# pySTEPS/pysteps

Hardware: AMD Instinct MI355X
Metric: Mpixels*leadsteps/s (LK+semilag) at 4096x4096 fp32 (higher is better)
Workload: dtype f32

## Files before the change

pysteps_amd/csrc/semilag.hip:

```cpp
#include <algorithm>
#include <cstdio>
#include <cstdlib>
#include <cstring>
#include <vector>

#include "common.h"

#pragma clang fp contract(off)

#include "semilag_device.h"

namespace psh {
namespace {

using namespace sl;

constexpr int kTileX = 64;
enum : int { kModeDirect = 0, kModePacked = 3, kModePacked2 = 4 };
constexpr int kDirectWaves = 8;
struct Fields {
  const float *u0, *v0, *p0;
  __amdgpu_buffer_rsrc_t ru, rv, rp;
  __amdgpu_buffer_rsrc_t ruv;
  __amdgpu_buffer_rsrc_t rpp;
// ... 353 lines not shown
        for (int j = 0; j < NPX; ++j) {
          mx[j] = px[j];
          my[j] = py[j];
          gx[j] = fx[j];
          gy[j] = fy[j];
          retreat(mx[j], gx[j], vix[j]);
          retreat(my[j], gy[j], viy[j]);
        }
        sample_at<NPX, ORDER, kVel, MODE, GEN>(F, mx, my, gx, gy, m, n, outval, su, sv, sp);
#pragma unroll
        for (int j = 0; j < NPX; ++j) {
          retreat(px[j], fx[j], su[j] * s);
          retreat(py[j], fy[j], sv[j] * s);
        }
        if (HAS_PRECIP && k == n_iter - 1) {
          sample_at<NPX, ORDER, kVel | kPrecip, MODE, GEN>(F, px, py, fx, fy, m, n, outval, su, sv, sp);
        } else {
          sample_at<NPX, ORDER, kVel, MODE, GEN>(F, px, py, fx, fy, m, n, outval, su, sv, sp);
        }
#pragma unroll
        for (int j = 0; j < NPX; ++j) {
          vix[j] = su[j] * half_s;
          viy[j] = sv[j] * half_s;
        }
      }
    } else {
      if (t > 0 || resume == 1) {
        sample_at<NPX, ORDER, kVel, MODE, GEN>(F, px, py, fx, fy, m, n, outval, su, sv, sp);
#pragma unroll
        for (int j = 0; j < NPX; ++j) {
          vix[j] = su[j] * s;
          viy[j] = sv[j] * s;
        }
      }
#pragma unroll
      for (int j = 0; j < NPX; ++j) {
        retreat(px[j], fx[j], vix[j]);
        retreat(py[j], fy[j], viy[j]);
      }
      if (HAS_PRECIP) {
        bool inside = true;
#pragma unroll
        for (int j = 0; j < NPX; ++j) inside = inside && wave_all_interior(px[j], py[j], m, n);
        if (ORDER == 1 && inside) {
          float v[NPX][4];
#pragma unroll
          for (int j = 0; j < NPX; ++j) {
            const unsigned off = static_cast<unsigned>(__mul24(py[j], n) + px[j]) << 2;
            v[j][0] = ld(F.p0, off);
            v[j][1] = ld(F.p0, off, 1);
            v[j][2] = ld(F.p0, off + static_cast<unsigned>(F.row_bytes));
            v[j][3] = ld(F.p0, off + static_cast<unsigned>(F.row_bytes), 1);
          }
#pragma unroll
          for (int j = 0; j < NPX; ++j)
            sp[j] = blend(make_weights(fx[j], fy[j]), v[j][0], v[j][1], v[j][2], v[j][3]);
          asm volatile("" ::: "memory");
        } else {
#pragma unroll
          for (int j = 0; j < NPX; ++j)
            sp[j] = ORDER == 3
                        ? sample_cubic<GEN>(F, px[j], py[j], fx[j], fy[j], m, n, outval)
                        : sample_precip_off_fast<(ORDER == 3 ? 1 : ORDER), GEN>(F.p0, px[j], py[j], fx[j], fy[j], m,
                                                                       n, outval, F.bmode);
        }
      }
    }
    if (HAS_PRECIP) {
#pragma unroll
      for (int j = 0; j < NPX; ++j) {
        sp[j] = lost(fx[j], fy[j]) ? lostval : sp[j];
        if (live[j]) {
          __builtin_nontemporal_store(sp[j], reinterpret_cast<float *>(reinterpret_cast<char *>(out) + opix[j]));
        }
      }
      out += static_cast<size_t>(rows) * n;
    }
  }

  if (disp != nullptr) {
#pragma unroll
    for (int j = 0; j < NPX; ++j) {
      if (!live[j]) continue;
      disp[static_cast<size_t>(y[j]) * n + x] =
          static_cast<double>(px[j]) - static_cast<double>(x) + static_cast<double>(fx[j]);
      disp[plane + static_cast<size_t>(y[j]) * n + x] =
          static_cast<double>(py[j]) - static_cast<double>(y[j]) + static_cast<double>(fy[j]);
    }
  }
}


typedef __attribute__((address_space(3))) void lds_void;
typedef __attribute__((address_space(3))) float lds_f32;
typedef __attribute__((address_space(3))) u32x4 lds_u32x4;
typedef __attribute__((address_space(3))) int lds_int;

__device__ __forceinline__ void win_barrier() { asm volatile("s_waitcnt lgkmcnt(0)\n\ts_barrier" ::: "memory"); }

__device__ __forceinline__ int rfl(int v) { return __builtin_amdgcn_readfirstlane(v); }

__device__ __forceinline__ int smin(int a, int b) {
  int r;
  asm("s_min_i32 %0, %1, %2" : "=s"(r) : "s"(a), "s"(b) : "scc");
  return r;
}
__device__ __forceinline__ int smax(int a, int b) {
  int r;
  asm("s_max_i32 %0, %1, %2" : "=s"(r) : "s"(a), "s"(b) : "scc");
  return r;
}

static unsigned long long *g_win_stats = nullptr;

template <int WAVES, int WW, int WH, int ROWS = 4, int OCC = 4>
struct WinCfg {
  static constexpr int kWaves = WAVES, kW = WW, kH = WH;
  static constexpr int kRows = ROWS;
  static constexpr int kOcc = OCC;
  static constexpr int kTileY = ROWS * WAVES;
  static constexpr unsigned kPitch4 = WW * 4u;
  static constexpr unsigned kPlaneBytes = WW * WH * 4u;
  static constexpr int kItems = WH * (WW / 4);
  static constexpr int kThreads = kTileX * WAVES;
  static constexpr unsigned kCtlVel = 16u * WAVES, kCtlFlag = kCtlVel + 8u;
  static constexpr unsigned kCtlTile = kCtlFlag + 12u;
  static constexpr int kCtlWords = 4 * WAVES + 2 + 3 + 3;
};
using Win8 = WinCfg<8, 96, 64>;

struct Window {
  unsigned uv, p;
  unsigned ctl;
  int ox, oy;
  int lo_x, hi_x, lo_y, hi_y;
  int edge;
  int fill16;
  unsigned long long *stats;
};

__device__ __forceinline__ void win_count(const Window &W, int which) {
  if (W.stats != nullptr && (threadIdx.x & 63) == 0) atomicAdd(W.stats + which, 1ull);
}

struct WinBox {
  int lox, hix, loy, hiy;
};
template <int kWinRows>
__device__ __forceinline__ WinBox win_corners(const int (&dxw)[kWinRows], const int (&dy)[kWinRows]) {
  const int xa = __builtin_amdgcn_readlane(dxw[0], 0), xb = __builtin_amdgcn_readlane(dxw[0], 63);
  const int xc = __builtin_amdgcn_readlane(dxw[kWinRows - 1], 0), xd = __builtin_amdgcn_readlane(dxw[kWinRows - 1], 63);
  const int ya = __builtin_amdgcn_readlane(dy[0], 0), yb = __builtin_amdgcn_readlane(dy[0], 63);
  const int yc = __builtin_amdgcn_readlane(dy[kWinRows - 1], 0), yd = __builtin_amdgcn_readlane(dy[kWinRows - 1], 63);
  return {smin(smin(xa, xb), smin(xc, xd)), smax(smax(xa, xb), smax(xc, xd)), smin(smin(ya, yb), smin(yc, yd)),
          smax(smax(ya, yb), smax(yc, yd))};
}

template <class C>
__device__ __forceinline__ void win_publish(const Window &W, int wave, const WinBox &bx, float vx_lane, float vy_lane) {
  typedef int i32x4 __attribute__((ext_vector_type(4)));
  typedef __attribute__((address_space(3))) i32x4 lds_i32x4;
  lds_int *ctl = (lds_int *)(size_t)W.ctl;
  *(lds_i32x4 *)(size_t)(W.ctl + 16u * wave) = i32x4{bx.lox, bx.hix, bx.loy, bx.hiy};
  if (wave == 0) {
    ctl[C::kCtlVel / 4 + 0] = __float_as_int(vx_lane);
    ctl[C::kCtlVel / 4 + 1] = __float_as_int(vy_lane);
  }
}

template <class C, bool GEN>
__device__ __forceinline__ void win_place_and_fill(const Fields &F, Window &W, bool force, int (&dxw)[C::kRows],
                                                    int (&dy)[C::kRows], float move_scale, int m, int n) {
  constexpr int kWinRows = C::kRows;
  lds_int *ctl = (lds_int *)(size_t)W.ctl;
  int ulox = 0x7fffffff, uhix = -0x7fffffff, uloy = 0x7fffffff, uhiy = -0x7fffffff;
#pragma unroll
  for (int w = 0; w < C::kWaves; ++w) {
    ulox = min(ulox, ctl[w * 4 + 0]);
    uhix = max(uhix, ctl[w * 4 + 1]);
    uloy = min(uloy, ctl[w * 4 + 2]);
    uhiy = max(uhiy, ctl[w * 4 + 3]);
  }
  const float wvx = __int_as_float(ctl[C::kCtlVel / 4 + 0]), wvy = __int_as_float(ctl[C::kCtlVel / 4 + 1]);
  const int bx0 = ulox, bx1 = uhix + 1, by0 = uloy, by1 = uhiy + 1;
  const int slack_x = max(C::kW - (bx1 - bx0 + 1), 0), slack_y = max(C::kH - (by1 - by0 + 1), 0);
  const int keep_x = wvx > 0.125f ? max(slack_x - 2, 0) : (wvx < -0.125f ? min(slack_x, 2) : slack_x / 2);
  const int keep_y = wvy > 0.125f ? max(slack_y - 2, 0) : (wvy < -0.125f ? min(slack_y, 2) : slack_y / 2);
  constexpr int kFar = 1 << 27;
  const int want_x = min(max(sat_add(W.ox, sat_sub(bx0, keep_x)), -kFar), kFar) & ~3;
  const int want_y = min(max(sat_add(W.oy, sat_sub(by0, keep_y)), -kFar), kFar);
  const int nox = rfl(GEN ? min(max(want_x, 0), n - C::kW) : want_x);
  const int noy = rfl(GEN ? min(max(want_y, 0), m - C::kH) : want_y);
  const bool edge = !GEN && (nox < 0 || nox + C::kW > n || noy < 0 || noy + C::kH > m);
  PSH_DASSERT((W.fill16 == 0 || (nox & 3) == 0) && (edge || (nox >= 0 && nox + C::kW <= n && noy >= 0 && noy + C::kH <= m)));
  const float mvx = fabsf(wvx) < 64.f ? fabsf(wvx) * move_scale + 2.f : 2.f, mvy = fabsf(wvy) < 64.f ? fabsf(wvy) * move_scale + 2.f : 2.f;
  const int gx = rfl(static_cast<int>(mvx)), gy = rfl(static_cast<int>(mvy));
  W.lo_x = wvx > 0.f ? gx : 1;
  W.hi_x = C::kW - 2 - (wvx > 0.f ? 1 : gx);
  W.lo_y = wvy > 0.f ? gy : 1;
  W.hi_y = C::kH - 2 - (wvy > 0.f ? 1 : gy);
  if (!force && nox == W.ox && noy == W.oy) return;
  win_count(W, 2);
  const int ddx = nox - W.ox, ddy = noy - W.oy;
#pragma unroll
  for (int j = 0; j < kWinRows; ++j) {
    dxw[j] = sat_sub(dxw[j], ddx);
    dy[j] = sat_sub(dy[j], ddy);
  }
  W.ox = nox;
  W.oy = noy;
  W.edge = edge ? 1 : 0;
  int tid = threadIdx.x;
  asm volatile("" : "+v"(tid));
  constexpr int kRounds = (C::kItems + C::kThreads - 1) / C::kThreads;
  u32x4 bu[kRounds], bv[kRounds], bp[kRounds];
  if (!edge) {
    const unsigned org = static_cast<unsigned>(noy) * static_cast<unsigned>(n) + static_cast<unsigned>(nox);
#pragma unroll
    for (int k = 0; k < kRounds; ++k) {
      const int item = min(tid + C::kThreads * k, C::kItems - 1);
      const int row = item / (C::kW / 4), c = item - row * (C::kW / 4);
      const int off = static_cast<int>((org + row * n + 4 * c) << 2);
      bu[k] = __builtin_amdgcn_raw_buffer_load_b128(F.ru, off, 0, 0);
      bv[k] = __builtin_amdgcn_raw_buffer_load_b128(F.rv, off, 0, 0);
      bp[k] = __builtin_amdgcn_raw_buffer_load_b128(F.rp, off, 0, 0);
    }
  } else if (!W.fill16) {
#pragma unroll
    for (int k = 0; k < kRounds; ++k) {
      const int item = min(tid + C::kThreads * k, C::kItems - 1);
      const int row = item / (C::kW / 4), c = item - row * (C::kW / 4);
      const int r = noy + row, x0 = nox + 4 * c;
      const int rv = min(max(r, 0), m - 1), rq = r == m ? m - 2 : rv;
      const unsigned base_v = static_cast<unsigned>(__mul24(rv, n)), base_q = static_cast<unsigned>(__mul24(rq, n));
      unsigned tu[4], tv[4], tq[4];
#pragma unroll
      for (int e = 0; e < 4; ++e) {
        const int x = x0 + e;
        const int xv = min(max(x, 0), n - 1), xq = x == n ? n - 2 : xv;
        tu[e] = __builtin_amdgcn_raw_buffer_load_b32(F.ru, static_cast<int>((base_v + xv) << 2), 0, 0);
        tv[e] = __builtin_amdgcn_raw_buffer_load_b32(F.rv, static_cast<int>((base_v + xv) << 2), 0, 0);
        tq[e] = __builtin_amdgcn_raw_buffer_load_b32(F.rp, static_cast<int>((base_q + xq) << 2), 0, 0);
      }
      bu[k] = u32x4{tu[0], tu[1], tu[2], tu[3]};
      bv[k] = u32x4{tv[0], tv[1], tv[2], tv[3]};
      bp[k] = u32x4{tq[0], tq[1], tq[2], tq[3]};
    }
  } else {
#pragma unroll
    for (int k = 0; k < kRounds; ++k) {
      const int item = min(tid + C::kThreads * k, C::kItems - 1);
      const int row = item / (C::kW / 4), c = item - row * (C::kW / 4);
      const int r = noy + row, x = nox + 4 * c;
      const int rv = min(max(r, 0), m - 1), rq = r == m ? m - 2 : rv;
      const int xi = min(max(x, 0), n - 4);
      const int off_v = static_cast<int>(static_cast<unsigned>(__mul24(rv, n) + xi) << 2);
      const int off_q = static_cast<int>(static_cast<unsigned>(__mul24(rq, n) + xi) << 2);
      u32x4 tu = __builtin_amdgcn_raw_buffer_load_b128(F.ru, off_v, 0, 0);
      u32x4 tv = __builtin_amdgcn_raw_buffer_load_b128(F.rv, off_v, 0, 0);
      u32x4 tq = __builtin_amdgcn_raw_buffer_load_b128(F.rp, off_q, 0, 0);
      if (x < 0) {
        tu = u32x4{tu.x, tu.x, tu.x, tu.x};
        tv = u32x4{tv.x, tv.x, tv.x, tv.x};
      } else if (x >= n) {
        tu = u32x4{tu.w, tu.w, tu.w, tu.w};
        tv = u32x4{tv.w, tv.w, tv.w, tv.w};
        tq = u32x4{tq.z, tq.z, tq.z, tq.z};
      }
      bu[k] = tu;
      bv[k] = tv;
      bp[k] = tq;
    }
  }
#pragma unroll
  for (int k = 0; k < kRounds; ++k) {
    const unsigned l = 16u * min(tid + C::kThreads * k, C::kItems - 1);
    *(lds_u32x4 *)(size_t)(W.uv + 2u * l) = u32x4{bu[k].x, bv[k].x, bu[k].y, bv[k].y};
    *(lds_u32x4 *)(size_t)(W.uv + 2u * l + 16u) = u32x4{bu[k].z, bv[k].z, bu[k].w, bv[k].w};
    *(lds_u32x4 *)(size_t)(W.p + l) = bp[k];
  }
}

template <class C, bool GEN>
__device__ __forceinline__ void win_update(const Fields &F, Window &W, int phase, bool force, int (&dxw)[C::kRows],
                                            int (&dy)[C::kRows], float vx_lane, float vy_lane, float move_scale, int m,
                                            int n) {
  const int lane = threadIdx.x & 63, wave = rfl(static_cast<int>(threadIdx.x >> 6));
  lds_int *ctl = (lds_int *)(size_t)W.ctl;
  const WinBox bx = win_corners(dxw, dy);
  const bool near = force || bx.lox < W.lo_x || bx.hix > W.hi_x || bx.loy < W.lo_y || bx.hiy > W.hi_y;
  if (lane == 0) {
    win_publish<C>(W, wave, bx, vx_lane, vy_lane);
    if (near) ctl[C::kCtlFlag / 4 + phase] = 1;
    if (wave == 0) ctl[C::kCtlFlag / 4 + (phase == 2 ? 0 : phase + 1)] = 0;
  }
  win_barrier();
  if (rfl(ctl[C::kCtlFlag / 4 + phase]) == 0) return;
  win_place_and_fill<C, GEN>(F, W, force, dxw, dy, move_scale, m, n);
  win_barrier();
}


template <class C, int WHAT, bool GEN>
__device__ __forceinline__ void win_sample(const Fields &F, const Window &W, const int (&dxw)[C::kRows],
                                            const int (&dy)[C::kRows], const f32x2 (&f)[C::kRows], int m, int n,
                                            float outval, f32x2 (&s_uv)[C::kRows], float (&sp)[C::kRows]) {
  constexpr int kWinRows = C::kRows;
  static_assert(kWinRows == 2 || kWinRows == 4, "rows per lane");
  constexpr bool kWithP = (WHAT & kPrecip) != 0;
  unsigned mx = static_cast<unsigned>(dxw[0]), my = static_cast<unsigned>(dy[0]);
#pragma unroll
  for (int j = 1; j < kWinRows; ++j) {
    mx = max(mx, static_cast<unsigned>(dxw[j]));
    my = max(my, static_cast<unsigned>(dy[j]));
  }
  const unsigned long long okx = __builtin_amdgcn_ballot_w64(mx <= static_cast<unsigned>(C::kW - 2));
  const unsigned long long oky = __builtin_amdgcn_ballot_w64(my <= static_cast<unsigned>(C::kH - 2));
  if ((okx & oky) == __builtin_amdgcn_ballot_w64(true)) {
    win_count(W, 0);
    f32x2 t[kWinRows][4];
    float rp[kWinRows][4];
#pragma unroll
    for (int j = 0; j < kWinRows; ++j) {
      const unsigned tx = __umul24(static_cast<unsigned>(dy[j]), static_cast<unsigned>(C::kW)) + static_cast<unsigned>(dxw[j]);
      PSH_DASSERT(static_cast<unsigned>(dxw[j]) <= static_cast<unsigned>(C::kW - 2) && static_cast<unsigned>(dy[j]) <= static_cast<unsigned>(C::kH - 2) &&
                  tx + C::kW + 1 < static_cast<unsigned>(C::kW * C::kH));
      const unsigned a = (tx << 3) + W.uv;
      asm volatile("ds_read_b64 %0, %4\n\tds_read_b64 %1, %4 offset:8\n\tds_read_b64 %2, %4 offset:%c5\n\t"
                   "ds_read_b64 %3, %4 offset:%c6"
                   : "=&v"(t[j][0]), "=&v"(t[j][1]), "=&v"(t[j][2]), "=&v"(t[j][3])
                   : "v"(a), "i"(2u * C::kPitch4), "i"(2u * C::kPitch4 + 8u));
      if (kWithP) {
        const unsigned ap = (tx << 2) + W.p;
        asm volatile("ds_read_b32 %0, %4\n\tds_read_b32 %1, %4 offset:4\n\tds_read_b32 %2, %4 offset:%c5\n\t"
                     "ds_read_b32 %3, %4 offset:%c6"
                     : "=&v"(rp[j][0]), "=&v"(rp[j][1]), "=&v"(rp[j][2]), "=&v"(rp[j][3])
                     : "v"(ap), "i"(C::kPitch4), "i"(C::kPitch4 + 4u));
      }
    }
    f32x2 w_mid[kWinRows];
    float w_00[kWinRows], w_11[kWinRows];
#ifndef PSH_WIN_NO_PAIR_WEIGHTS
    constexpr bool kPairs = !GEN && kWithP && kWinRows == 4;
    f32x2 q00[2], q01[2], q10[2], q11[2];
    if constexpr (kPairs) {
#pragma unroll
      for (int pr = 0; pr < 2; ++pr) {
        const f32x2 fa = f[2 * pr], fb = f[2 * pr + 1];
        const f32x2 ga = 1.f - fa, gb = 1.f - fb;
        float a00, b00, a01, b01, a10, b10, a11, b11;
        asm volatile("v_mul_f32 %0, %1, %2" : "=v"(a00) : "v"(ga.x), "v"(ga.y));
        asm volatile("v_mul_f32 %0, %1, %2" : "=v"(b00) : "v"(gb.x), "v"(gb.y));
        asm volatile("v_mul_f32 %0, %1, %2" : "=v"(a01) : "v"(fa.x), "v"(ga.y));
        asm volatile("v_mul_f32 %0, %1, %2" : "=v"(b01) : "v"(fb.x), "v"(gb.y));
        asm volatile("v_mul_f32 %0, %1, %2" : "=v"(a10) : "v"(fa.y), "v"(ga.x));
        asm volatile("v_mul_f32 %0, %1, %2" : "=v"(b10) : "v"(fb.y), "v"(gb.x));
        asm volatile("v_mul_f32 %0, %1, %2" : "=v"(a11) : "v"(fa.x), "v"(fa.y));
        asm volatile("v_mul_f32 %0, %1, %2" : "=v"(b11) : "v"(fb.x), "v"(fb.y));
        q00[pr] = f32x2{a00, b00};
        q01[pr] = f32x2{a01, b01};
        q10[pr] = f32x2{a10, b10};
        q11[pr] = f32x2{a11, b11};
        asm volatile("" : "+v"(q00[pr]), "+v"(q01[pr]), "+v"(q10[pr]), "+v"(q11[pr]));
      }
    } else
#else
    constexpr bool kPairs = false;
#endif
    if constexpr (!GEN) {
#pragma unroll
      for (int j = 0; j < kWinRows; ++j) {
        const f32x2 g = 1.f - f[j];
        w_mid[j] = f[j] * g.yx;
        asm volatile("v_mul_f32 %0, %1, %2" : "=v"(w_00[j]) : "v"(g.x), "v"(g.y));
        asm volatile("v_mul_f32 %0, %1, %2" : "=v"(w_11[j]) : "v"(f[j].x), "v"(f[j].y));
        asm volatile("" ::"v"(w_mid[j]));
      }
    }
#define PSH_TIE4(A, J) "+v"(A[J][0]), "+v"(A[J][1]), "+v"(A[J][2]), "+v"(A[J][3])
#ifndef PSH_WIN_NO_STAGED_WAIT
    if constexpr (kWinRows == 4 && !GEN) {
      if (kWithP) {
        asm volatile("s_waitcnt lgkmcnt(15)" : PSH_TIE4(t, 0), PSH_TIE4(t, 1));
        asm volatile("" : PSH_TIE4(rp, 0), PSH_TIE4(rp, 1));
      } else {
        asm volatile("s_waitcnt lgkmcnt(8)" : PSH_TIE4(t, 0), PSH_TIE4(t, 1));
      }
      __builtin_amdgcn_sched_barrier(0);
    } else
#endif
    if constexpr (kWinRows == 4) {
      asm volatile("s_waitcnt lgkmcnt(0)" : PSH_TIE4(t, 0), PSH_TIE4(t, 1), PSH_TIE4(t, 2), PSH_TIE4(t, 3));
      if (kWithP) asm volatile("" : PSH_TIE4(rp, 0), PSH_TIE4(rp, 1), PSH_TIE4(rp, 2), PSH_TIE4(rp, 3));
    } else {
      asm volatile("s_waitcnt lgkmcnt(0)" : PSH_TIE4(t, 0), PSH_TIE4(t, 1));
      if (kWithP) asm volatile("" : PSH_TIE4(rp, 0), PSH_TIE4(rp, 1));
    }
#ifndef PSH_WIN_NO_PAIR_WEIGHTS
    if constexpr (kPairs) {
#pragma unroll
      for (int pr = 0; pr < 2; ++pr) {
        const int a = 2 * pr, b = 2 * pr + 1;
#ifndef PSH_WIN_NO_STAGED_WAIT
        if (pr == 1) {
          __builtin_amdgcn_sched_barrier(0);
          asm volatile("s_waitcnt lgkmcnt(0)" : PSH_TIE4(t, 2), PSH_TIE4(t, 3));
          asm volatile("" : PSH_TIE4(rp, 2), PSH_TIE4(rp, 3));
          __builtin_amdgcn_sched_barrier(0);
        }
#endif
        f32x2 acc = t[a][0] * f32x2{q00[pr].x, q00[pr].x};
        acc = __builtin_elementwise_fma(f32x2{q01[pr].x, q01[pr].x}, t[a][1], acc);
        acc = __builtin_elementwise_fma(f32x2{q10[pr].x, q10[pr].x}, t[a][2], acc);
        acc = __builtin_elementwise_fma(f32x2{q11[pr].x, q11[pr].x}, t[a][3], acc);
        s_uv[a] = acc;
        acc = t[b][0] * f32x2{q00[pr].y, q00[pr].y};
        acc = __builtin_elementwise_fma(f32x2{q01[pr].y, q01[pr].y}, t[b][1], acc);
        acc = __builtin_elementwise_fma(f32x2{q10[pr].y, q10[pr].y}, t[b][2], acc);
        acc = __builtin_elementwise_fma(f32x2{q11[pr].y, q11[pr].y}, t[b][3], acc);
        s_uv[b] = acc;
        f32x2 ps = q00[pr] * f32x2{rp[a][0], rp[b][0]};
        ps = __builtin_elementwise_fma(q01[pr], f32x2{rp[a][1], rp[b][1]}, ps);
        ps = __builtin_elementwise_fma(q10[pr], f32x2{rp[a][2], rp[b][2]}, ps);
        ps = __builtin_elementwise_fma(q11[pr], f32x2{rp[a][3], rp[b][3]}, ps);
        sp[a] = ps.x;
        sp[b] = ps.y;
      }
    } else
#endif
#pragma unroll
    for (int j = 0; j < kWinRows; ++j) {
#ifndef PSH_WIN_NO_STAGED_WAIT
      if constexpr (kWinRows == 4 && !GEN) {
        if (j == 2) {
          __builtin_amdgcn_sched_barrier(0);
          asm volatile("s_waitcnt lgkmcnt(0)" : PSH_TIE4(t, 2), PSH_TIE4(t, 3));
          if (kWithP) asm volatile("" : PSH_TIE4(rp, 2), PSH_TIE4(rp, 3));
          __builtin_amdgcn_sched_barrier(0);
        }
      }
#endif
      f32x2 w00, wmid, w11;
      if constexpr (GEN) {
        const f32x2 g = 1.f - f[j];
        w00 = g * g.yx;
        wmid = f[j] * g.yx;
        w11 = f[j] * f[j].yx;
      } else {
        w00 = f32x2{w_00[j], w_00[j]};
        wmid = w_mid[j];
        w11 = f32x2{w_11[j], w_11[j]};
      }
      f32x2 acc = t[j][0] * f32x2{w00.x, w00.x};
      acc = __builtin_elementwise_fma(f32x2{wmid.x, wmid.x}, t[j][1], acc);
      acc = __builtin_elementwise_fma(f32x2{wmid.y, wmid.y}, t[j][2], acc);
      acc = __builtin_elementwise_fma(f32x2{w11.x, w11.x}, t[j][3], acc);
      s_uv[j] = acc;
      if (kWithP) sp[j] = fmaf(w11.x, rp[j][3], fmaf(wmid.y, rp[j][2], fmaf(wmid.x, rp[j][1], w00.x * rp[j][0])));
    }
#undef PSH_TIE4
    if constexpr (kWithP && !GEN) {
      if (W.edge) {
#pragma unroll
        for (int j = 0; j < kWinRows; ++j) {
          const int X = sat_add(W.ox, dxw[j]), Y = sat_add(W.oy, dy[j]);
          const bool outside = X < 0 || Y < 0 || X > n - 1 || Y > m - 1 || (X == n - 1 && f[j].x > 0.f) || (Y == m - 1 && f[j].y > 0.f);
          sp[j] = outside ? outval : sp[j];
        }
      }
    }
  } else {
    win_count(W, 1);
    int X[kWinRows], Y[kWinRows];
    float sfx[kWinRows], sfy[kWinRows], ssu[kWinRows], ssv[kWinRows], ssp[kWinRows];
#pragma unroll
    for (int j = 0; j < kWinRows; ++j) {
      X[j] = sat_add(W.ox, dxw[j]);
      Y[j] = sat_add(W.oy, dy[j]);
      sfx[j] = f[j].x;
      sfy[j] = f[j].y;
      ssp[j] = 0.f;
    }
    sample_at<kWinRows, 1, WHAT, kModeDirect, GEN>(F, X, Y, sfx, sfy, m, n, outval, ssu, ssv, ssp);
#pragma unroll
    for (int j = 0; j < kWinRows; ++j) {
      s_uv[j] = f32x2{ssu[j], ssv[j]};
      if (kWithP) sp[j] = ssp[j];
    }
  }
}

__device__ __forceinline__ void retreat_xy(int &PX, int &PY, f32x2 &f, f32x2 w) {
  const f32x2 t = f - w;
  int kx, ky;
  asm("v_cvt_flr_i32_f32 %0, %1" : "=v"(kx) : "v"(t.x));
  asm("v_cvt_flr_i32_f32 %0, %1" : "=v"(ky) : "v"(t.y));
  PX = sat_add(PX, kx);
  PY = sat_add(PY, ky);
  f = f32x2{__builtin_amdgcn_fractf(t.x), __builtin_amdgcn_fractf(t.y)};
}

__device__ __attribute__((noinline)) int win_next_slot(unsigned *queue, int home, int tiles_per_xcd, const int *order) {
  for (int i = 0; i < kNumXcd; ++i) {
    const int k = (home + i) & (kNumXcd - 1);
    if (__hip_atomic_load(queue + k, __ATOMIC_RELAXED, __HIP_MEMORY_SCOPE_AGENT) >= static_cast<unsigned>(tiles_per_xcd)) continue;
    const unsigned l = __hip_atomic_fetch_add(queue + k, 1u, __ATOMIC_RELAXED, __HIP_MEMORY_SCOPE_AGENT);
    if (l < static_cast<unsigned>(tiles_per_xcd)) {
      const int t = order[l * kNumXcd + k];
      if (t >= 0) return t;
    }
  }
  return -1;
}

template <class C, bool GEN, bool PERSIST>
__global__ __launch_bounds__(C::kThreads, C::kOcc) void semilag_window(
    const float *__restrict__ precip, const float *__restrict__ vel, float *__restrict__ out_base, double *__restrict__ disp,
    const float *__restrict__ scale, float first_scale, int m, int n, int T, int n_iter, int resume, float outval,
    int row0, int rows, int bmode, int tiles_x, int n_tiles, int tiles_per_xcd, float guard,
    const int *__restrict__ order, unsigned *__restrict__ queue, unsigned long long *__restrict__ stats) {
  constexpr int kWinRows = C::kRows;
  const size_t plane = static_cast<size_t>(m) * n;
  Fields F;
  F.u0 = vel;
  F.v0 = vel + plane;
  F.p0 = precip;
  const int plane_bytes = static_cast<int>(plane * sizeof(float));
  F.ru = __builtin_amdgcn_make_buffer_rsrc(const_cast<float *>(vel), 0, plane_bytes, 0x00020000);
  F.rv = __builtin_amdgcn_make_buffer_rsrc(const_cast<float *>(vel + plane), 0, plane_bytes, 0x00020000);
  F.rp = __builtin_amdgcn_make_buffer_rsrc(const_cast<float *>(precip), 0, plane_bytes, 0x00020000);
  F.ruv = F.ru;
  F.rpp = F.ru;
  F.row_bytes = n * static_cast<int>(sizeof(float));
  F.coef = nullptr;
  F.cpad = 0;
  F.sorder = 3;
  F.minval = 0.f;
  F.bmode = bmode;

  __shared__ __attribute__((aligned(16))) float win_planes[3 * C::kW * C::kH];
  __shared__ __attribute__((aligned(16))) int win_ctl[C::kCtlWords];
  const int lane = threadIdx.x & (kTileX - 1);
  const float move_scale = guard * static_cast<float>(n_iter);
  const float lostval = (bmode == kModeNearest || bmode == kModeGridConstant) ? __builtin_nanf("") : outval;
  const int home = static_cast<int>(blockIdx.x) & (kNumXcd - 1);
  int tile = PERSIST ? -1 : order[blockIdx.x];
  int next = -1;
  if (PERSIST && threadIdx.x == 0) next = win_next_slot(queue, home, tiles_per_xcd, order);

  for (;;) {
    if (PERSIST) {
      if (threadIdx.x == 0) win_ctl[C::kCtlTile / 4] = next;
      __syncthreads();
      tile = rfl(win_ctl[C::kCtlTile / 4]);
    }
    if (tile < 0) break;
    if (PERSIST && threadIdx.x == 0) next = win_next_slot(queue, home, tiles_per_xcd, order);
    PSH_DASSERT(tile < n_tiles);
    const int xt = (tile % tiles_x) * kTileX + lane;
    const int yt = row0 + (tile / tiles_x) * C::kTileY + static_cast<int>(threadIdx.x / kTileX) * kWinRows;
    const int x = min(xt, n - 1);
    float *out = out_base;
#ifndef PSH_WIN_MASKED_STORES
    const int out_plane_bytes = static_cast<int>(static_cast<unsigned>(__mul24(rows, n)) * 4u);
#endif
    Window W;
    W.uv = static_cast<unsigned>(reinterpret_cast<size_t>((lds_void *)win_planes));
    W.p = W.uv + 2u * C::kPlaneBytes;
    W.ctl = static_cast<unsigned>(reinterpret_cast<size_t>((lds_void *)win_ctl));
    W.ox = W.oy = 0;
    W.lo_x = W.lo_y = 0;
    W.hi_x = W.hi_y = 0;
    W.edge = 0;
    W.fill16 = ((n & 3) == 0 && (plane & 3) == 0 &&
                ((reinterpret_cast<uintptr_t>(vel) | reinterpret_cast<uintptr_t>(precip)) & 15) == 0)
                   ? 1
                   : 0;
    W.stats = stats;
    if (threadIdx.x < 3) win_ctl[C::kCtlFlag / 4 + threadIdx.x] = 0;

    int y[kWinRows], dxw[kWinRows], dy[kWinRows];
    f32x2 f[kWinRows], vi[kWinRows], s_uv[kWinRows];
    float sp[kWinRows];
    bool live[kWinRows];
    unsigned opix[kWinRows];
#pragma unroll
    for (int j = 0; j < kWinRows; ++j) {
      live[j] = xt < n && yt + j < row0 + rows;
      y[j] = min(yt + j, m - 1);
      opix[j] = static_cast<unsigned>(__mul24(y[j] - row0, n) + x) << 2;
#ifndef PSH_WIN_MASKED_STORES
      if (!live[j]) opix[j] = 0xfffffff0u;
#endif
      int px = x, py = y[j];
      float ifx = 0.f, ify = 0.f, ivx = 0.f, ivy = 0.f;
      if (resume) {
        split_displacement(disp[static_cast<size_t>(y[j]) * n + x], px, ifx);
        split_displacement(disp[plane + static_cast<size_t>(y[j]) * n + x], py, ify);
      }
      if (resume != 1) {
        const unsigned pix = static_cast<unsigned>(__mul24(y[j], n) + x) << 2;
        ivx = ld(F.u0, pix) * first_scale;
        ivy = ld(F.v0, pix) * first_scale;
      }
      dxw[j] = px;
      dy[j] = py;
      f[j] = f32x2{ifx, ify};
      vi[j] = f32x2{ivx, ivy};
      sp[j] = 0.f;
    }
    __syncthreads();
    int phase = 0;
    win_update<C, GEN>(F, W, phase, true, dxw, dy, 0.5f * vi[0].x, 0.5f * vi[0].y, move_scale, m, n);
    phase = 1;
    if (resume == 1) {
      win_sample<C, kVel, GEN>(F, W, dxw, dy, f, m, n, outval, s_uv, sp);
      const float s0 = scale[0];
#pragma unroll
      for (int j = 0; j < kWinRows; ++j) vi[j] = s_uv[j] * s0;
    }
#pragma unroll
    for (int j = 0; j < kWinRows; ++j) vi[j] = vi[j] * 0.5f;

    for (int t = 0; t < T; ++t) {
      const float s = scale[t];
      const float half_s = 0.5f * s;
      for (int k = 0; k < n_iter; ++k) {
        int mxw[kWinRows], my[kWinRows];
        f32x2 g[kWinRows];
#pragma unroll
        for (int j = 0; j < kWinRows; ++j) {
          mxw[j] = dxw[j];
          my[j] = dy[j];
          g[j] = f[j];
          retreat_xy(mxw[j], my[j], g[j], vi[j]);
        }
        win_sample<C, kVel, GEN>(F, W, mxw, my, g, m, n, outval, s_uv, sp);
#pragma unroll
        for (int j = 0; j < kWinRows; ++j) retreat_xy(dxw[j], dy[j], f[j], s_uv[j] * s);
        if (k == n_iter - 1) {
          win_sample<C, kVel | kPrecip, GEN>(F, W, dxw, dy, f, m, n, outval, s_uv, sp);
        } else {
          win_sample<C, kVel, GEN>(F, W, dxw, dy, f, m, n, outval, s_uv, sp);
        }
#pragma unroll
        for (int j = 0; j < kWinRows; ++j) vi[j] = s_uv[j] * half_s;
      }
#pragma unroll
      for (int j = 0; j < kWinRows; ++j) {
        const float val = lost(f[j].x, f[j].y) ? lostval : sp[j];
#ifndef PSH_WIN_MASKED_STORES
        __builtin_amdgcn_raw_buffer_store_b32(__float_as_uint(val), __builtin_amdgcn_make_buffer_rsrc(out, 0, out_plane_bytes, 0x00020000),
                                              static_cast<int>(opix[j]), 0, 2 );
#else
        if (live[j]) __builtin_nontemporal_store(val, reinterpret_cast<float *>(reinterpret_cast<char *>(out) + opix[j]));
#endif
      }
      out += static_cast<size_t>(rows) * n;
      if (t + 1 < T) {
        win_update<C, GEN>(F, W, phase, false, dxw, dy, vi[0].x, vi[0].y, move_scale, m, n);
        phase = phase == 2 ? 0 : phase + 1;
      }
    }

    if (disp != nullptr) {
#pragma unroll
      for (int j = 0; j < kWinRows; ++j) {
        if (!live[j]) continue;
        disp[static_cast<size_t>(y[j]) * n + x] = static_cast<double>(sat_add(W.ox, dxw[j])) - static_cast<double>(x) + static_cast<double>(f[j].x);
        disp[plane + static_cast<size_t>(y[j]) * n + x] = static_cast<double>(sat_add(W.oy, dy[j])) - static_cast<double>(y[j]) + static_cast<double>(f[j].y);
      }
    }
    if (!PERSIST) return;
  }
  if (PERSIST && threadIdx.x == 0) {
    if (__hip_atomic_fetch_add(queue + kNumXcd, 1u, __ATOMIC_ACQ_REL, __HIP_MEMORY_SCOPE_AGENT) == gridDim.x - 1) {
      for (int i = 0; i <= kNumXcd; ++i) __hip_atomic_store(queue + i, 0u, __ATOMIC_RELAXED, __HIP_MEMORY_SCOPE_AGENT);
    }
  }
}

static bool window_shape(int m, int n) { return n >= Win8::kW && m >= Win8::kH; }

bool semilag_window_eligible(const SemilagArgs &a) {
  return a.precip != nullptr && a.order == 1 && a.n_iter >= 1 && window_shape(a.m, a.n) &&
         static_cast<size_t>(a.m) * a.n * sizeof(float) < 0xfffffff0ull;
}

struct WinOrder {
  int tiles_x = 0, tiles_y = 0, tile_h = 0, mode = -1;
  int *dev = nullptr;
  void *stage = nullptr;
};
static WinOrder g_win_orders[8];
static int g_win_orders_next = 0;
static unsigned *g_win_queue = nullptr;
static unsigned g_win_queue_turn = 0;
constexpr int kQueueRing = 16;
[[maybe_unused]] static const int g_win_hook = at_shutdown([] { g_win_orders_next = g_win_queue_turn = 0; });

static std::vector<int> win_order_table(int tiles_x, int tiles_y, int tile_h, int mode) {
  const int n_tiles = tiles_x * tiles_y, per = (n_tiles + kNumXcd - 1) / kNumXcd;
  const bool cells = (mode & 1) && tiles_x % kNumXcd == 0 && tiles_y % kNumXcd == 0;
  std::vector<int> table(static_cast<size_t>(per) * kNumXcd, -1);
  for (int k = 0; k < kNumXcd; ++k) {
    std::vector<int> mine;
    for (int l = 0; l < per; ++l) {
      int tile;
      if (cells) {
        const int cw = tiles_x / kNumXcd, ch = tiles_y / kNumXcd, per_cell = cw * ch;
        const int cy = l / per_cell, r = l - cy * per_cell;
        const int cx = (k + kNumXcd - cy) & (kNumXcd - 1);
        tile = (cy * ch + r / cw) * tiles_x + cx * cw + r % cw;
      } else {
        tile = k * per + l;
      }
      if (tile < n_tiles) mine.push_back(tile);
    }
    if (mode & 2) {
      auto ring = [&](int tile) {
        const int tx = tile % tiles_x, ty = tile / tiles_x;
        const int d = std::min(std::min(tx, tiles_x - 1 - tx) * kTileX, std::min(ty, tiles_y - 1 - ty) * tile_h);
        return std::min(d, 192) / 32;
      };
      std::stable_sort(mine.begin(), mine.end(), [&](int a, int b) { return ring(a) < ring(b); });
    }
    for (size_t l = 0; l < mine.size(); ++l) table[l * kNumXcd + k] = mine[l];
  }
  return table;
}

static const int *win_order(int tiles_x, int tiles_y, int tile_h, int mode, hipStream_t stream) {
  for (const WinOrder &o : g_win_orders)
    if (o.dev != nullptr && o.tiles_x == tiles_x && o.tiles_y == tiles_y && o.tile_h == tile_h && o.mode == mode) return o.dev;
  WinOrder &o = g_win_orders[g_win_orders_next];
  g_win_orders_next = (g_win_orders_next + 1) % 8;
  const std::vector<int> table = win_order_table(tiles_x, tiles_y, tile_h, mode);
  const size_t bytes = table.size() * sizeof(int);
  if (o.dev != nullptr && hipStreamSynchronize(stream) != hipSuccess) return nullptr;
  float *src = nullptr;
  const float *ring_dev = nullptr;
  if (bytes > kConstSlotFloats * sizeof(float)) {
    if (persistent_pinned(&o.stage, bytes) != PSH_OK) return nullptr;
    src = static_cast<float *>(o.stage);
  } else if (const_slot(&src, &ring_dev) != PSH_OK) {
    return nullptr;
  }
  std::memcpy(src, table.data(), bytes);
  if (persistent_device(&o.dev, bytes) != PSH_OK) return nullptr;
  if (hipMemcpyAsync(o.dev, src, bytes, hipMemcpyHostToDevice, stream) != hipSuccess) {
    persistent_free(reinterpret_cast<void **>(&o.dev));
    return nullptr;
  }
  o.tiles_x = tiles_x;
  o.tiles_y = tiles_y;
  o.tile_h = tile_h;
  o.mode = mode;
  return o.dev;
}

static int env_int(const char *name, int fallback) {
  const char *e = std::getenv(name);
  return e ? std::atoi(e) : fallback;
}

template <class C>
static hipError_t launch_window(const SemilagArgs &a, hipStream_t stream) {
  const int tiles_x = (a.n + kTileX - 1) / kTileX;
  const int tiles_y = (a.rows + C::kTileY - 1) / C::kTileY;
  const int n_tiles = tiles_x * tiles_y;
  const int tiles_per_xcd = (n_tiles + kNumXcd - 1) / kNumXcd;
  static const bool want_stats = std::getenv("PYSTEPS_HIP_SL_STATS") != nullptr;
  static const float guard = std::getenv("PYSTEPS_HIP_SL_GUARD") ? static_cast<float>(std::atof(std::getenv("PYSTEPS_HIP_SL_GUARD"))) : 2.0f;
  static const int order_mode = (env_int("PYSTEPS_HIP_SL_CELLS", 1) ? 1 : 0) | (env_int("PYSTEPS_HIP_SL_RINGS", 1) ? 2 : 0);
  static const int persist = env_int("PYSTEPS_HIP_SL_PERSIST", 0);
  const int *order = win_order(tiles_x, tiles_y, C::kTileY, order_mode, stream);
  if (order == nullptr) return hipErrorOutOfMemory;
  unsigned *queue = nullptr;
  const int resident = persist > 1 ? persist : psh::ctx().cu_count * (4 * C::kOcc / C::kWaves);
  int grid_x = tiles_per_xcd * kNumXcd;
  if (persist && (grid_x > resident || persist > 1)) {
    if (g_win_queue == nullptr) {
      if (persistent_device(&g_win_queue, kQueueRing * 16 * sizeof(unsigned)) != PSH_OK) return hipErrorOutOfMemory;
      if (hipMemsetAsync(g_win_queue, 0, kQueueRing * 16 * sizeof(unsigned), stream) != hipSuccess) return hipErrorUnknown;
    }
    queue = g_win_queue + 16 * (g_win_queue_turn++ % kQueueRing);
    grid_x = resident;
  }
  const dim3 grid(grid_x), block(C::kThreads);
  if (want_stats) {
    (void)persistent_device(&g_win_stats, 4 * sizeof(unsigned long long));
    if (g_win_stats != nullptr) (void)hipMemsetAsync(g_win_stats, 0, 4 * sizeof(unsigned long long), stream);
  }
#define PSH_WIN_LAUNCH(GEN, PERSIST)                                                                               \
  hipLaunchKernelGGL((semilag_window<C, GEN, PERSIST>), grid, block, 0, stream, a.precip, a.vel, a.out, a.disp, a.scale, \
                     a.first_scale, a.m, a.n, a.T, a.n_iter, a.resume, a.outval, a.row0, a.rows, a.bmode, tiles_x,      \
                     n_tiles, tiles_per_xcd, guard, order, queue, g_win_stats)
  if (a.bmode != 0) {
    if (queue != nullptr) PSH_WIN_LAUNCH(true, true); else PSH_WIN_LAUNCH(true, false);
  } else {
    if (queue != nullptr) PSH_WIN_LAUNCH(false, true); else PSH_WIN_LAUNCH(false, false);
  }
#undef PSH_WIN_LAUNCH
  const hipError_t e = hipGetLastError();
  if (e == hipSuccess && want_stats && g_win_stats != nullptr) {
    unsigned long long h[4] = {0, 0, 0, 0};
    if (hipMemcpyAsync(h, g_win_stats, sizeof(h), hipMemcpyDeviceToHost, stream) == hipSuccess &&
        hipStreamSynchronize(stream) == hipSuccess)
      std::fprintf(stderr, "semilag_window<%d waves x %d rows>: %dx%d T=%d: wave-passes through the window %llu, through the gathers %llu, "
                   "window fills (per wave) %llu (%d tiles on %d workgroups x %d lead steps)\n", C::kWaves, C::kRows, a.m, a.n, a.T,
                   h[0], h[1], h[2], n_tiles, grid_x, a.T);
  }
  return e;
}

template <int NPX, int MODE>
static hipError_t launch_variant(const SemilagArgs &a, hipStream_t stream) {
  constexpr int kWaves = kDirectWaves;
  const int tile_y = kWaves * NPX;
  const int tiles_x = (a.n + kTileX - 1) / kTileX;
  const int tiles_y = (a.rows + tile_y - 1) / tile_y;
  const int n_tiles = tiles_x * tiles_y;
  const int tiles_per_xcd = (n_tiles + kNumXcd - 1) / kNumXcd;
  const dim3 grid(tiles_per_xcd * kNumXcd), block(kTileX * kWaves);
#define PSH_SL_LAUNCH(ORDER, HASP, GEN)                                                         \
  hipLaunchKernelGGL((semilag_fused<NPX, ORDER, HASP, MODE, GEN>), grid, block, 0, stream,      \
                     a.precip, a.vel, a.vel_packed, a.field_pairs, a.out, a.disp, a.scale, a.first_scale, a.m, a.n, \
                     a.T,                                                                                  \
                     a.n_iter, a.resume, a.outval, a.row0, a.rows, a.coef, a.minval, a.bmode, a.coef_pad | (a.spline_order << 8),  \
                     tiles_x, n_tiles, tiles_per_xcd)
  if (a.precip == nullptr) {
    PSH_SL_LAUNCH(1, false, false);
  } else if (a.order == 0) {
    if (a.bmode != 0) {
      PSH_SL_LAUNCH(0, true, true);
    } else {
      PSH_SL_LAUNCH(0, true, false);
    }
  } else if (a.order == 3) {
    if (a.bmode != 0) {
      PSH_SL_LAUNCH(3, true, true);
    } else {
      PSH_SL_LAUNCH(3, true, false);
    }
  } else if (a.bmode != 0) {
    PSH_SL_LAUNCH(1, true, true);
  } else {
    PSH_SL_LAUNCH(1, true, false);
  }
#undef PSH_SL_LAUNCH
  return hipGetLastError();
}

}

static int g_semilag_variant = [] {
  const char *e = std::getenv("PYSTEPS_HIP_SL_VARIANT");
  return e ? std::atoi(e) : 0;
}();

void set_semilag_variant(int v) { g_semilag_variant = v; }

constexpr long long kWindowMinPasses = 2;

bool semilag_uses_window(const SemilagArgs &a) {
  if (!semilag_window_eligible(a)) return false;
  if (g_semilag_variant == 12) return true;
  return g_semilag_variant == 0 && static_cast<long long>(a.T) * a.n_iter >= kWindowMinPasses;
}

bool semilag_window_shape(int m, int n) { return window_shape(m, n); }

int semilag_kernel_choice(int m, int n, int T, int n_iter, int order, bool has_field) {
  SemilagArgs a{};
  static float dummy[4] __attribute__((aligned(16)));
  a.precip = has_field ? dummy : nullptr;
  a.vel = dummy;
  a.m = m;
  a.n = n;
  a.T = T;
  a.n_iter = n_iter;
  a.order = order;
  if (semilag_uses_window(a)) return 12;
  if (semilag_wants_field_pairs(a)) return 7;
  if (semilag_wants_packed(a)) return 5;
  return 1;
}

hipError_t launch_semilag(const SemilagArgs &a, hipStream_t stream) {
  if (semilag_uses_window(a)) return launch_window<Win8>(a, stream);
  if (a.vel_packed != nullptr && a.field_pairs != nullptr && a.order == 1) return launch_variant<1, kModePacked2>(a, stream);
  if (a.vel_packed != nullptr) return launch_variant<1, kModePacked>(a, stream);
  return launch_variant<1, kModeDirect>(a, stream);
}

bool semilag_wants_packed(const SemilagArgs &a) {
  return !semilag_uses_window(a) && (g_semilag_variant == 0 || g_semilag_variant == 5 || g_semilag_variant == 7) &&
         static_cast<uint64_t>(a.m) * static_cast<uint64_t>(a.n) < (1ull << 29) &&
         static_cast<long long>(a.T) * (a.n_iter > 0 ? a.n_iter : 1) >= 8;
}
bool semilag_wants_field_pairs(const SemilagArgs &a) {
  return (g_semilag_variant == 0 || g_semilag_variant == 7) && semilag_wants_packed(a) && a.precip != nullptr &&
         a.order == 1 && a.T >= 8;
}

hipError_t launch_pack_field_rows(const float *precip, float *pairs, int m, int n, hipStream_t stream) {
  hipLaunchKernelGGL(pack_field_rows, dim3((n + 1023) / 1024, m), dim3(256), 0, stream, precip, pairs, m, n);
  return hipGetLastError();
}

hipError_t launch_pack_velocity(const float *vel, float *uv, size_t plane, hipStream_t stream) {
  const size_t threads = (plane + 3) / 4;
  hipLaunchKernelGGL(pack_velocity, dim3(static_cast<unsigned>((threads + 255) / 256)), dim3(256), 0, stream, vel, uv,
                     plane);
  return hipGetLastError();
}

}
```

Baseline: 279,000.

## Fuse last-iteration midpoint and endpoint LDS samples into one staggered substep

Adds a fused substep for the final semi-Lagrangian iteration in the non-generated 4-row window path. It interleaves the midpoint velocity blend, the retreat, and the endpoint velocity and precip LDS reads in row pairs, using explicit lgkmcnt waits so LDS latency overlaps with arithmetic. If any lane leaves the window, the endpoint is resampled through the gather path. This adds inline-asm complexity and register pressure, and the speculative reads are wasted on fallback. It also reworks the displacement address calculation.

```diff
diff --git a/pysteps_amd/csrc/semilag.hip b/pysteps_amd/csrc/semilag.hip
--- a/pysteps_amd/csrc/semilag.hip
+++ b/pysteps_amd/csrc/semilag.hip
@@ -679,6 +679,30 @@
 
 
 template <class C, int WHAT, bool GEN>
+__device__ __forceinline__ void win_gather(const Fields &F, const Window &W, const int (&dxw)[C::kRows],
+                                            const int (&dy)[C::kRows], const f32x2 (&f)[C::kRows], int m, int n,
+                                            float outval, f32x2 (&s_uv)[C::kRows], float (&sp)[C::kRows]) {
+  constexpr int kWinRows = C::kRows;
+  win_count(W, 1);
+  int X[kWinRows], Y[kWinRows];
+  float sfx[kWinRows], sfy[kWinRows], ssu[kWinRows], ssv[kWinRows], ssp[kWinRows];
+#pragma unroll
+  for (int j = 0; j < kWinRows; ++j) {
+    X[j] = sat_add(W.ox, dxw[j]);
+    Y[j] = sat_add(W.oy, dy[j]);
+    sfx[j] = f[j].x;
+    sfy[j] = f[j].y;
+    ssp[j] = 0.f;
+  }
+  sample_at<kWinRows, 1, WHAT, kModeDirect, GEN>(F, X, Y, sfx, sfy, m, n, outval, ssu, ssv, ssp);
+#pragma unroll
+  for (int j = 0; j < kWinRows; ++j) {
+    s_uv[j] = f32x2{ssu[j], ssv[j]};
+    if ((WHAT & kPrecip) != 0) sp[j] = ssp[j];
+  }
+}
+
+template <class C, int WHAT, bool GEN>
 __device__ __forceinline__ void win_sample(const Fields &F, const Window &W, const int (&dxw)[C::kRows],
                                             const int (&dy)[C::kRows], const f32x2 (&f)[C::kRows], int m, int n,
                                             float outval, f32x2 (&s_uv)[C::kRows], float (&sp)[C::kRows]) {
@@ -877,6 +901,174 @@
   f = f32x2{__builtin_amdgcn_fractf(t.x), __builtin_amdgcn_fractf(t.y)};
 }
 
+template <class C>
+__device__ __forceinline__ bool win_inside(const int (&dxw)[C::kRows], const int (&dy)[C::kRows]) {
+  unsigned mx = static_cast<unsigned>(dxw[0]), my = static_cast<unsigned>(dy[0]);
+#pragma unroll
+  for (int j = 1; j < C::kRows; ++j) {
+    mx = max(mx, static_cast<unsigned>(dxw[j]));
+    my = max(my, static_cast<unsigned>(dy[j]));
+  }
+  const unsigned long long okx = __builtin_amdgcn_ballot_w64(mx <= static_cast<unsigned>(C::kW - 2));
+  const unsigned long long oky = __builtin_amdgcn_ballot_w64(my <= static_cast<unsigned>(C::kH - 2));
+  return (okx & oky) == __builtin_amdgcn_ballot_w64(true);
+}
+
+template <class C>
+__device__ __forceinline__ bool win_substep(const Fields &F, const Window &W, const int (&mxw)[4], const int (&my)[4],
+                                             const f32x2 (&g)[4], int (&dxw)[4], int (&dy)[4], f32x2 (&f)[4], float s,
+                                             int m, int n, float outval, f32x2 (&s_uv)[4], float (&sp)[4]) {
+  static_assert(C::kRows == 4, "rows per lane");
+  const unsigned long long all = __builtin_amdgcn_ballot_w64(true);
+  win_count(W, 0);
+  asm volatile("" : "+s"(s));
+  unsigned long long ok = all;
+  f32x2 t[4][4], u[4][4];
+  float rp[4][4];
+  f32x2 w_mid[4];
+  float w_00[4], w_11[4];
+  f32x2 q00[2], q01[2], q10[2], q11[2];
+#define PSH_READ_UV(D, A)                                                                                          \
+  asm volatile("ds_read_b64 %0, %4\n\tds_read_b64 %1, %4 offset:8\n\tds_read_b64 %2, %4 offset:%c5\n\t"          \
+               "ds_read_b64 %3, %4 offset:%c6"                                                                    \
+               : "=&v"(D[0]), "=&v"(D[1]), "=&v"(D[2]), "=&v"(D[3])                                               \
+               : "v"(A), "i"(2u * C::kPitch4), "i"(2u * C::kPitch4 + 8u))
+#define PSH_READ_P(D, A)                                                                                           \
+  asm volatile("ds_read_b32 %0, %4\n\tds_read_b32 %1, %4 offset:4\n\tds_read_b32 %2, %4 offset:%c5\n\t"          \
+               "ds_read_b32 %3, %4 offset:%c6"                                                                    \
+               : "=&v"(D[0]), "=&v"(D[1]), "=&v"(D[2]), "=&v"(D[3])                                               \
+               : "v"(A), "i"(C::kPitch4), "i"(C::kPitch4 + 4u))
+#define PSH_TIE4(A, J) "+v"(A[J][0]), "+v"(A[J][1]), "+v"(A[J][2]), "+v"(A[J][3])
+#define PSH_WAIT_UV(N, A, PR)                                                \
+  __builtin_amdgcn_sched_barrier(0);                                         \
+  asm volatile("s_waitcnt lgkmcnt(" #N ")" : PSH_TIE4(A, 2 * PR), PSH_TIE4(A, 2 * PR + 1)); \
+  __builtin_amdgcn_sched_barrier(0)
+#define PSH_WAIT_UVP(N, PR)                                                  \
+  __builtin_amdgcn_sched_barrier(0);                                         \
+  asm volatile("s_waitcnt lgkmcnt(" #N ")" : PSH_TIE4(u, 2 * PR), PSH_TIE4(u, 2 * PR + 1)); \
+  asm volatile("" : PSH_TIE4(rp, 2 * PR), PSH_TIE4(rp, 2 * PR + 1));         \
+  __builtin_amdgcn_sched_barrier(0)
+#pragma unroll
+  for (int j = 0; j < 4; ++j) {
+    const unsigned tx = __umul24(static_cast<unsigned>(my[j]), static_cast<unsigned>(C::kW)) + static_cast<unsigned>(mxw[j]);
+    PSH_DASSERT(tx + C::kW + 1 < static_cast<unsigned>(C::kW * C::kH));
+    const unsigned a = (tx << 3) + W.uv;
+    PSH_READ_UV(t[j], a);
+  }
+#pragma unroll
+  for (int j = 0; j < 4; ++j) {
+    const f32x2 h = 1.f - g[j];
+    w_mid[j] = g[j] * h.yx;
+    asm volatile("v_mul_f32 %0, %1, %2" : "=v"(w_00[j]) : "v"(h.x), "v"(h.y));
+    asm volatile("v_mul_f32 %0, %1, %2" : "=v"(w_11[j]) : "v"(g[j].x), "v"(g[j].y));
+    asm volatile("" ::"v"(w_mid[j]));
+  }
+  auto mid_blend = [&](int pr) __attribute__((always_inline)) {
+#pragma unroll
+    for (int j = 2 * pr; j < 2 * pr + 2; ++j) {
+      f32x2 acc = t[j][0] * f32x2{w_00[j], w_00[j]};
+      acc = __builtin_elementwise_fma(f32x2{w_mid[j].x, w_mid[j].x}, t[j][1], acc);
+      acc = __builtin_elementwise_fma(f32x2{w_mid[j].y, w_mid[j].y}, t[j][2], acc);
+      acc = __builtin_elementwise_fma(f32x2{w_11[j], w_11[j]}, t[j][3], acc);
+      retreat_xy(dxw[j], dy[j], f[j], acc * s);
+    }
+  };
+  auto end_issue = [&](int pr) __attribute__((always_inline)) {
+    const int a = 2 * pr, b = 2 * pr + 1;
+    const unsigned mx = max(static_cast<unsigned>(dxw[a]), static_cast<unsigned>(dxw[b]));
+    const unsigned mmy = max(static_cast<unsigned>(dy[a]), static_cast<unsigned>(dy[b]));
+    ok &= __builtin_amdgcn_ballot_w64(mx <= static_cast<unsigned>(C::kW - 2));
+    ok &= __builtin_amdgcn_ballot_w64(mmy <= static_cast<unsigned>(C::kH - 2));
+#pragma unroll
+    for (int j = a; j <= b; ++j) {
+      const unsigned tx = min(__umul24(static_cast<unsigned>(dy[j]), static_cast<unsigned>(C::kW)) + static_cast<unsigned>(dxw[j]),
+                              static_cast<unsigned>(C::kW * C::kH - C::kW - 2));
+      PSH_DASSERT(tx + C::kW + 1 < static_cast<unsigned>(C::kW * C::kH));
+      const unsigned auv = (tx << 3) + W.uv, ap = (tx << 2) + W.p;
+      PSH_READ_UV(u[j], auv);
+      PSH_READ_P(rp[j], ap);
+    }
+    const f32x2 fa = f[a], fb = f[b];
+    const f32x2 ga = 1.f - fa, gb = 1.f - fb;
+    float a00, b00, a01, b01, a10, b10, a11, b11;
+    asm volatile("v_mul_f32 %0, %1, %2" : "=v"(a00) : "v"(ga.x), "v"(ga.y));
+    asm volatile("v_mul_f32 %0, %1, %2" : "=v"(b00) : "v"(gb.x), "v"(gb.y));
+    asm volatile("v_mul_f32 %0, %1, %2" : "=v"(a01) : "v"(fa.x), "v"(ga.y));
+    asm volatile("v_mul_f32 %0, %1, %2" : "=v"(b01) : "v"(fb.x), "v"(gb.y));
+    asm volatile("v_mul_f32 %0, %1, %2" : "=v"(a10) : "v"(fa.y), "v"(ga.x));
+    asm volatile("v_mul_f32 %0, %1, %2" : "=v"(b10) : "v"(fb.y), "v"(gb.x));
+    asm volatile("v_mul_f32 %0, %1, %2" : "=v"(a11) : "v"(fa.x), "v"(fa.y));
+    asm volatile("v_mul_f32 %0, %1, %2" : "=v"(b11) : "v"(fb.x), "v"(fb.y));
+    q00[pr] = f32x2{a00, b00};
+    q01[pr] = f32x2{a01, b01};
+    q10[pr] = f32x2{a10, b10};
+    q11[pr] = f32x2{a11, b11};
+    asm volatile("" : "+v"(q00[pr]), "+v"(q01[pr]), "+v"(q10[pr]), "+v"(q11[pr]));
+  };
+  auto end_blend = [&](int pr) __attribute__((always_inline)) {
+    const int a = 2 * pr, b = 2 * pr + 1;
+    f32x2 acc = u[a][0] * f32x2{q00[pr].x, q00[pr].x};
+    acc = __builtin_elementwise_fma(f32x2{q01[pr].x, q01[pr].x}, u[a][1], acc);
+    acc = __builtin_elementwise_fma(f32x2{q10[pr].x, q10[pr].x}, u[a][2], acc);
+    acc = __builtin_elementwise_fma(f32x2{q11[pr].x, q11[pr].x}, u[a][3], acc);
+    s_uv[a] = acc;
+    acc = u[b][0] * f32x2{q00[pr].y, q00[pr].y};
+    acc = __builtin_elementwise_fma(f32x2{q01[pr].y, q01[pr].y}, u[b][1], acc);
+    acc = __builtin_elementwise_fma(f32x2{q10[pr].y, q10[pr].y}, u[b][2], acc);
+    acc = __builtin_elementwise_fma(f32x2{q11[pr].y, q11[pr].y}, u[b][3], acc);
+    s_uv[b] = acc;
+    f32x2 ps = q00[pr] * f32x2{rp[a][0], rp[b][0]};
+    ps = __builtin_elementwise_fma(q01[pr], f32x2{rp[a][1], rp[b][1]}, ps);
+    ps = __builtin_elementwise_fma(q10[pr], f32x2{rp[a][2], rp[b][2]}, ps);
+    ps = __builtin_elementwise_fma(q11[pr], f32x2{rp[a][3], rp[b][3]}, ps);
+    sp[a] = ps.x;
+    sp[b] = ps.y;
+    asm volatile("" : "+v"(s_uv[a]), "+v"(s_uv[b]), "+v"(sp[a]), "+v"(sp[b]));
+  };
+#ifndef PSH_WIN_NO_STAGGER
+  PSH_WAIT_UV(8, t, 0);
+  mid_blend(0);
+  end_issue(0);
+  PSH_WAIT_UV(15, t, 1);
+  mid_blend(1);
+  end_issue(1);
+  PSH_WAIT_UVP(15, 0);
+  end_blend(0);
+  PSH_WAIT_UVP(0, 1);
+  end_blend(1);
+#else
+  PSH_WAIT_UV(8, t, 0);
+  mid_blend(0);
+  PSH_WAIT_UV(0, t, 1);
+  mid_blend(1);
+  end_issue(0);
+  end_issue(1);
+  PSH_WAIT_UVP(15, 0);
+  end_blend(0);
+  PSH_WAIT_UVP(0, 1);
+  end_blend(1);
+#endif
+#undef PSH_READ_UV
+#undef PSH_READ_P
+#undef PSH_TIE4
+#undef PSH_WAIT_UV
+#undef PSH_WAIT_UVP
+  if (ok != all) {
+    win_count(W, 3);
+    return false;
+  }
+  win_count(W, 0);
+  if (W.edge) {
+#pragma unroll
+    for (int j = 0; j < 4; ++j) {
+      const int X = sat_add(W.ox, dxw[j]), Y = sat_add(W.oy, dy[j]);
+      const bool outside = X < 0 || Y < 0 || X > n - 1 || Y > m - 1 || (X == n - 1 && f[j].x > 0.f) || (Y == m - 1 && f[j].y > 0.f);
+      sp[j] = outside ? outval : sp[j];
+    }
+  }
+  return true;
+}
+
 __device__ __attribute__((noinline)) int win_next_slot(unsigned *queue, int home, int tiles_per_xcd, const int *order) {
   for (int i = 0; i < kNumXcd; ++i) {
     const int k = (home + i) & (kNumXcd - 1);
@@ -1012,13 +1204,33 @@
           g[j] = f[j];
           retreat_xy(mxw[j], my[j], g[j], vi[j]);
         }
-        win_sample<C, kVel, GEN>(F, W, mxw, my, g, m, n, outval, s_uv, sp);
-#pragma unroll
-        for (int j = 0; j < kWinRows; ++j) retreat_xy(dxw[j], dy[j], f[j], s_uv[j] * s);
-        if (k == n_iter - 1) {
-          win_sample<C, kVel | kPrecip, GEN>(F, W, dxw, dy, f, m, n, outval, s_uv, sp);
+        constexpr bool kFast = !GEN && kWinRows == 4;
+        if constexpr (kFast) {
+          const bool last = k == n_iter - 1;
+          bool done = false;
+          if (last && win_inside<C>(mxw, my)) {
+            done = win_substep<C>(F, W, mxw, my, g, dxw, dy, f, s, m, n, outval, s_uv, sp);
+          } else {
+            win_sample<C, kVel, GEN>(F, W, mxw, my, g, m, n, outval, s_uv, sp);
+#pragma unroll
+            for (int j = 0; j < kWinRows; ++j) retreat_xy(dxw[j], dy[j], f[j], s_uv[j] * s);
+          }
+          if (!done) {
+            if (last) {
+              win_gather<C, kVel | kPrecip, GEN>(F, W, dxw, dy, f, m, n, outval, s_uv, sp);
+            } else {
+              win_sample<C, kVel, GEN>(F, W, dxw, dy, f, m, n, outval, s_uv, sp);
+            }
+          }
         } else {
-          win_sample<C, kVel, GEN>(F, W, dxw, dy, f, m, n, outval, s_uv, sp);
+          win_sample<C, kVel, GEN>(F, W, mxw, my, g, m, n, outval, s_uv, sp);
+#pragma unroll
+          for (int j = 0; j < kWinRows; ++j) retreat_xy(dxw[j], dy[j], f[j], s_uv[j] * s);
+          if (k == n_iter - 1) {
+            win_sample<C, kVel | kPrecip, GEN>(F, W, dxw, dy, f, m, n, outval, s_uv, sp);
+          } else {
+            win_sample<C, kVel, GEN>(F, W, dxw, dy, f, m, n, outval, s_uv, sp);
+          }
         }
 #pragma unroll
         for (int j = 0; j < kWinRows; ++j) vi[j] = s_uv[j] * half_s;
@@ -1041,11 +1253,14 @@
     }
 
     if (disp != nullptr) {
+      int xe = x, ye = yt;
+      asm volatile("" : "+v"(xe), "+v"(ye));
 #pragma unroll
       for (int j = 0; j < kWinRows; ++j) {
         if (!live[j]) continue;
-        disp[static_cast<size_t>(y[j]) * n + x] = static_cast<double>(sat_add(W.ox, dxw[j])) - static_cast<double>(x) + static_cast<double>(f[j].x);
-        disp[plane + static_cast<size_t>(y[j]) * n + x] = static_cast<double>(sat_add(W.oy, dy[j])) - static_cast<double>(y[j]) + static_cast<double>(f[j].y);
+        const int yj = min(ye + j, m - 1);
+        disp[static_cast<size_t>(yj) * n + xe] = static_cast<double>(sat_add(W.ox, dxw[j])) - static_cast<double>(xe) + static_cast<double>(f[j].x);
+        disp[plane + static_cast<size_t>(yj) * n + xe] = static_cast<double>(sat_add(W.oy, dy[j])) - static_cast<double>(yj) + static_cast<double>(f[j].y);
       }
     }
     if (!PERSIST) return;
@@ -1185,8 +1400,8 @@
     if (hipMemcpyAsync(h, g_win_stats, sizeof(h), hipMemcpyDeviceToHost, stream) == hipSuccess &&
         hipStreamSynchronize(stream) == hipSuccess)
       std::fprintf(stderr, "semilag_window<%d waves x %d rows>: %dx%d T=%d: wave-passes through the window %llu, through the gathers %llu, "
-                   "window fills (per wave) %llu (%d tiles on %d workgroups x %d lead steps)\n", C::kWaves, C::kRows, a.m, a.n, a.T,
-                   h[0], h[1], h[2], n_tiles, grid_x, a.T);
+                   "window fills (per wave) %llu, end-point samples redone %llu (%d tiles on %d workgroups x %d lead steps)\n",
+                   C::kWaves, C::kRows, a.m, a.n, a.T, h[0], h[1], h[2], h[3], n_tiles, grid_x, a.T);
   }
   return e;
 }
```

Result: slower. 271,800 (-2.6%).
